# ygjwd12345/UCD

Hardware: AMD Instinct MI355X
Metric: images/sec (whole node) per UCD train step, VOC 15-5 step-1, 513^2 bs=24 (higher is better)
Workload: dtype bf16

## Files before the change

### include/ucd_hip.h

```cpp
#ifndef UCD_HIP_H
#define UCD_HIP_H

#include <stddef.h>
#include <stdint.h>

#ifdef __cplusplus
extern "C" {
#endif

#define UCD_VERSION 100

typedef void* ucd_stream_t;
typedef void* ucd_comm_t;

enum ucd_dtype { UCD_F32 = 0, UCD_BF16 = 1 };
enum ucd_act { UCD_ACT_IDENTITY = 0, UCD_ACT_LEAKY_RELU = 1, UCD_ACT_ELU = 2  };
#define UCD_ACT_MASK 0xff
#define UCD_NORM_ABS_GAMMA 0x100
enum ucd_pixcon_precision { UCD_PIXCON_F32 = 0, UCD_PIXCON_F16 = 1, UCD_PIXCON_F16_SPLIT = 2 };
enum ucd_error {
  UCD_OK = 0,
  UCD_EINVAL = -1,
  UCD_EALIGN = -2,
  UCD_EWORKSPACE = -3,
// ... 247 lines not shown
  const void* residual;  int ldr;
  int out_act;  float out_slope;
  float* partial;
  int accumulate;
  int taps, H, W, dilation;
  const void* side2;  int ld2;
  int stride;
  float* stat_acc;  const float* stat_shift;  float* stat_acc2;
  int stat_rep;
} ucd_conv1x1_desc;

int ucd_conv1x1_row_tiles(int M);
int ucd_conv1x1_stat_replicas(int M);
size_t ucd_conv1x1_stats_partial_bytes(int M, int C);
int ucd_conv1x1(const ucd_conv1x1_desc* desc, ucd_stream_t stream);

int ucd_conv1x1_stats_finalize(const float* partial, int M, int C, const float* weight, float* running_mean,
                               float* running_var, float momentum, float eps, float* buf, float* pack, int flags,
                               ucd_stream_t stream);

int ucd_abn_reduce_partials(const float* partial, int tiles, int C, float* sums, float* sums_copy, const float* weight,
                            int flags, ucd_stream_t stream);

size_t ucd_conv1x1_wgrad_workspace_bytes(int M, int N, int K);
int ucd_conv1x1_wgrad(const void* dy, int ld_dy, const void* a, int lda, int M, int N, int K,
                      const float* in_mean, const float* in_scale, const float* in_shift, int in_act, float in_slope,
                      void* dw, void* workspace, size_t workspace_bytes, ucd_stream_t stream);

int ucd_abn_sync_finalize(const float* gathered, int world, int M, int C, const float* weight, float* running_mean,
                          float* running_var, float momentum, float eps, float* buf, int flags, ucd_stream_t stream);
// ... 84 lines not shown
```

### ucd_amd/csrc/conv1x1.hip

```cpp
#include "common.h"
#include "abn_finalize.h"

namespace ucd {
namespace {

typedef float f32x16 __attribute__((ext_vector_type(16)));
typedef __bf16 bf16x8 __attribute__((ext_vector_type(8)));
typedef __hip_bfloat16 bf16;

constexpr int kThreads = 256;
constexpr int kBM = 128;

constexpr int kBK = 64;
constexpr int kDbStages = 2;
constexpr int kLwStages = 3;

struct Args {
  const bf16* A; int lda;
  const bf16* W; int ldw;
  bf16* Y; int ldy;
  int M, N, K;
  const float *in_mean, *in_scale, *in_shift; int in_act; float in_slope;
  const float *out_mean, *out_scale, *out_shift, *out_invstd;
  const bf16* R; int ldr;
  const bf16* Z; int ldz;
  int out_act; float out_slope;
  float* partial;
  int accumulate;
  int tiles_m, tiles_n;
  int param_off;
  int iH, iW, dil;
  int stride, oW, ohw;
  int a_rows;
  int tiles128;
  float* stat_acc;
  const float* stat_shift;
  float* stat_acc2;
  int stat_rep;
};

__device__ __forceinline__ float act_rt(float z, float slope) { return z > 0.f ? z : z * slope; }
__device__ __forceinline__ float act_grad_rt(float z, float slope) { return z > 0.f ? 1.f : slope; }

__device__ __forceinline__ int swz_fn(int row) { return (row >> 1) & 7; }
__device__ __forceinline__ int swz(int row, int slot) { return row * 128 + ((slot ^ swz_fn(row)) << 4); }

typedef __attribute__((address_space(1))) const void* gptr_t;
typedef __attribute__((address_space(3))) void* lptr_t;


template <int OUT> constexpr int kEpilogueBarriers = 4 + (OUT >= 2 ? 2 : 0);
template <int OUT, int HALVES> constexpr int kEpilogueBarriersH = 2 * HALVES + (OUT >= 2 ? 2 : 0);

__device__ __forceinline__ void live_taps(int m0, int m1, int ohw, int oW, int iH, int dil, int& tap0, int& ntap) {
  tap0 = 0; ntap = 9;
  if (dil <= 1 || m1 - m0 >= ohw) return;
  const int first = m0 % ohw, last = (m1 - 1) % ohw;
  int ymin = first / oW, ymax = last / oW;
  if (first > last) { ymin = 0; ymax = iH - 1; }
  if (ymax < dil) { tap0 = 3; ntap -= 3; }
  if (ymin >= iH - dil) ntap -= 3;
}

template <int BN, bool PRO, int OUT, bool CONV3 = false, bool DB = false>
__global__ __launch_bounds__(kThreads, DB ? 2 : ((PRO || OUT >= 3) && BN == 128 ? 3 : 4)) void conv1x1_kernel(Args p) {
  static_assert(!DB || !PRO, "the double-buffered form has no input transform");
  constexpr int kStage = (kBM + BN) * kBK * 2;
  constexpr int WN = BN / 2;
  constexpr int TN = WN / 32;
  extern __shared__ __attribute__((aligned(1024))) unsigned char smem[];
  unsigned char* As = smem;
  unsigned char* Bs = smem + kBM * kBK * 2;
  float* Ps = reinterpret_cast<float*>(smem + p.param_off);

  const int xcd = blockIdx.x & 7, j = blockIdx.x >> 3;
  const int tm = (j / p.tiles_n) * 8 + xcd, tn = j % p.tiles_n;
  if (tm >= p.tiles_m) return;
  const int m0 = tm * kBM, n0 = tn * BN;
  const int tid = threadIdx.x, lane = tid & 63, wave = __builtin_amdgcn_readfirstlane(tid >> 6);
  const int wm = wave >> 1, wn = wave & 1;

// ... 6 lines not shown
      for (int r = 0; r < 16; ++r) acc[a][b][r] = 0.f;

  constexpr int RPC = 1024 / (kBK * 2), SPR = kBK / 8;
  constexpr int CA = kBM / RPC / 4, CB = BN / RPC / 4;
  const bf16* ga[CA];
  const bf16* gb[CB];
  int py[CA], px[CA], pimg[CA], pslot[CA];
#pragma unroll
  for (int i = 0; i < CA; ++i) {
    const int row = RPC * (wave * CA + i) + lane / SPR;
    const int slot = ((lane % SPR) ^ swz_fn(row)) << 3;
    ga[i] = p.A + (size_t)min(m0 + row, p.M - 1) * p.lda + slot;
    if (CONV3 || p.stride > 1) {
      const int m = m0 + row;
      const int mm = min(m, p.M - 1);
      const int b = mm / p.ohw, rem = mm - b * p.ohw;
      const int oy = rem / p.oW, ox = rem - oy * p.oW;
      py[i] = m < p.M ? oy * p.stride : -(1 << 20);
      px[i] = ox * p.stride;
      pimg[i] = b * p.iH * p.iW;
      pslot[i] = slot;
      if (!CONV3) ga[i] = p.A + (size_t)(pimg[i] + oy * p.stride * p.iW + px[i]) * p.lda + slot;
    }
  }
#pragma unroll
  for (int i = 0; i < CB; ++i) {
    const int row = RPC * (wave * CB + i) + lane / SPR;
    gb[i] = p.W + (size_t)(n0 + row) * p.ldw + (((lane % SPR) ^ swz_fn(row)) << 3);
  }
  const int ks = tid & 7, srow = tid >> 3;
  const bf16* arow[4];
#pragma unroll
  for (int i = 0; i < 4; ++i) arow[i] = p.A + (size_t)min(m0 + srow + 32 * i, p.M - 1) * p.lda + ks * 8;

  if (PRO) {
    for (int k = tid; k < p.K; k += kThreads) {
      Ps[k] = p.in_mean[k];
      Ps[p.K + k] = p.in_scale[k];
      Ps[2 * p.K + k] = p.in_shift ? p.in_shift[k] : 0.f;
    }
    __syncthreads();
  }
  const int fr = lane & 31, fh = lane >> 5;
  const int kpt = p.K / kBK;
  int tap0 = 0, ntap = 9;
  if (CONV3 && p.stride == 1) live_taps(m0, min(m0 + kBM, p.M), p.ohw, p.oW, p.iH, p.dil, tap0, ntap);
  const int nk = CONV3 ? ntap * kpt : kpt;
  uint4 ra[4];
  if (PRO) {
#pragma unroll
    for (int i = 0; i < 4; ++i) ra[i] = *reinterpret_cast<const uint4*>(arow[i]);
  }
  const auto rsW = __builtin_amdgcn_make_buffer_rsrc((void*)p.W, 0, (int)((size_t)p.N * p.ldw * 2), 0x00020000);
  const auto rsA1 = __builtin_amdgcn_make_buffer_rsrc((void*)p.A, 0, (int)((size_t)p.a_rows * p.lda * 2), 0x00020000);
  unsigned boff[CB], a1off[CA];
#pragma unroll
  for (int i = 0; i < CB; ++i) boff[i] = (unsigned)((const char*)gb[i] - (const char*)p.W);
#pragma unroll
  for (int i = 0; i < CA; ++i) a1off[i] = (unsigned)((const char*)ga[i] - (const char*)p.A);
  const auto rsA = __builtin_amdgcn_make_buffer_rsrc((void*)p.A, 0, CONV3 ? (int)((size_t)p.a_rows * p.lda * 2) : 0, 0x00020000);
  constexpr unsigned kOOB = 0x7FFFFFF0u;
  unsigned aoff[CA];
  int atap = -1;
  auto set_tap = [&](int tap) {
    const int dy = (tap / 3 - 1) * p.dil, dx = (tap % 3 - 1) * p.dil;
#pragma unroll
    for (int i = 0; i < CA; ++i) {
      const int yy = py[i] + dy, xx = px[i] + dx;
      const bool ok = (unsigned)yy < (unsigned)p.iH && (unsigned)xx < (unsigned)p.iW;
      aoff[i] = ok ? (unsigned)(((pimg[i] + yy * p.iW + xx) * p.lda + pslot[i]) * 2) : kOOB;
    }
    atap = tap;
  };
  auto fill3 = [&](int kb, unsigned char* Ad, unsigned char* Bd) {
    const int kt = CONV3 ? kb / kpt : 0, tap = tap0 + kt;
    const int k0 = (kb - kt * kpt) * kBK;
    if (CONV3) {
      if (tap != atap) set_tap(tap);
#pragma unroll
      for (int i = 0; i < CA; ++i)
        __builtin_amdgcn_raw_ptr_buffer_load_lds(rsA, (lptr_t)(Ad + (wave * CA + i) * 1024), 16, (int)aoff[i], k0 * 2, 0, 0);
    } else {
#pragma unroll
      for (int i = 0; i < CA; ++i)
        __builtin_amdgcn_raw_ptr_buffer_load_lds(rsA1, (lptr_t)(Ad + (wave * CA + i) * 1024), 16, (int)a1off[i], k0 * 2, 0, 0);
    }
#pragma unroll
    for (int i = 0; i < CB; ++i)
      __builtin_amdgcn_raw_ptr_buffer_load_lds(rsW, (lptr_t)(Bd + (wave * CB + i) * 1024), 16, (int)boff[i], (tap * p.K + k0) * 2, 0, 0);
  };
  if (DB) {
#pragma unroll
    for (int st = 0; st < kDbStages - 1; ++st)
      if (st < nk) fill3(st, As + st * kStage, Bs + st * kStage);
  }
  for (int kb = 0; kb < nk; ++kb) {
    const int kt = CONV3 ? kb / kpt : 0, tap = tap0 + kt;
    const int k0 = (kb - kt * kpt) * kBK;
    const int wk0 = CONV3 ? tap * p.K + k0 : k0;
    if (kb) {
      if (DB) {
        asm volatile("s_waitcnt lgkmcnt(0)" ::: "memory");
        __builtin_amdgcn_s_barrier();
      } else {
        __syncthreads();
      }
    }
    const unsigned char* Ac = As + (DB ? (kb & (kDbStages - 1)) * kStage : 0);
    const unsigned char* Bc = Bs + (DB ? (kb & (kDbStages - 1)) * kStage : 0);
    if (DB) {
      if (kb + kDbStages - 1 < nk) {
        const int st = (kb + kDbStages - 1) & (kDbStages - 1);
// ... 76 lines not shown
#pragma unroll
        for (int a = 0; a < 2; ++a) af[a] = *reinterpret_cast<const bf16x8*>(Ac + swz(wm * 64 + a * 32 + fr, 2 * kk + fh));
#pragma unroll
        for (int b = 0; b < TN; ++b) bfr[b] = *reinterpret_cast<const bf16x8*>(Bc + swz(wn * WN + b * 32 + fr, 2 * kk + fh));
#pragma unroll
        for (int a = 0; a < 2; ++a)
#pragma unroll
          for (int b = 0; b < TN; ++b) acc[a][b] = __builtin_amdgcn_mfma_f32_32x32x16_bf16(af[a], bfr[b], acc[a][b], 0, 0, 0);
      }
    }
  }

#include "conv1x1_epilogue.inc"
}

template <int BM, int BN, int OUT, bool CONV3>
__global__ __launch_bounds__(BM == 64 ? 384 : BM * 4, (BM + BN) * kBK * 2 * kLwStages > 80 * 1024 ? 1 : 2) void conv_lw_kernel(Args p) {
  static_assert(BM == 64 || BM == 128 || BM == 256, "64-, 128- or 256-row workgroup tiles");
  static_assert(BM != 64 || BN == 64, "the 64-row form runs its epilogue on 128 threads: 64-column tiles");
  constexpr int NC = BM / 32, NL = BM == 64 ? 4 : BM / 32;
  constexpr int kStage = (BM + BN) * kBK * 2;
  constexpr int WN = BN / 2, TN = WN / 32;
  extern __shared__ __attribute__((aligned(1024))) unsigned char smem[];
  unsigned char* As = smem;
  unsigned char* Bs = smem + BM * kBK * 2;
  const int xcd = blockIdx.x & 7, j = blockIdx.x >> 3;
  const int tmw = (j / p.tiles_n) * 8 + xcd, tn = j % p.tiles_n;
  if (tmw >= p.tiles_m) return;
  const int m0w = tmw * BM, n0 = tn * BN;
  const int tid = threadIdx.x, lane = tid & 63, wave = __builtin_amdgcn_readfirstlane(tid >> 6);
  const int kpt = p.K / kBK;
  int tap0 = 0, ntap = 9;
  if (CONV3 && p.stride == 1) live_taps(m0w, min(m0w + BM, p.M), p.ohw, p.oW, p.iH, p.dil, tap0, ntap);
  const int nk = CONV3 ? ntap * kpt : kpt;

  if (wave >= NC) {
    const int lw = wave - NC;
    const int m0 = m0w;
    constexpr int RPC = 1024 / (kBK * 2), SPR = kBK / 8;
    constexpr int CA = BM / RPC / NL, CB = BN / RPC / NL;
    int py[CA], px[CA], pimg[CA], pslot[CA];
    unsigned a1off[CA], boff[CB];
#pragma unroll
    for (int i = 0; i < CA; ++i) {
      const int row = RPC * (lw * CA + i) + lane / SPR;
      const int slot = ((lane % SPR) ^ swz_fn(row)) << 3;
      a1off[i] = (unsigned)(((size_t)min(m0 + row, p.M - 1) * p.lda + slot) * 2);
      if (CONV3 || p.stride > 1) {
        const int m = m0 + row;
        const int mm = min(m, p.M - 1);
        const int b = mm / p.ohw, rem = mm - b * p.ohw;
        const int oy = rem / p.oW, ox = rem - oy * p.oW;
        py[i] = m < p.M ? oy * p.stride : -(1 << 20);
        px[i] = ox * p.stride;
        pimg[i] = b * p.iH * p.iW;
        pslot[i] = slot;
        if (!CONV3) a1off[i] = (unsigned)(((size_t)(pimg[i] + oy * p.stride * p.iW + px[i]) * p.lda + slot) * 2);
      }
    }
#pragma unroll
    for (int i = 0; i < CB; ++i) {
      const int row = RPC * (lw * CB + i) + lane / SPR;
      boff[i] = (unsigned)(((size_t)(n0 + row) * p.ldw + (((lane % SPR) ^ swz_fn(row)) << 3)) * 2);
    }
    const auto rsW = __builtin_amdgcn_make_buffer_rsrc((void*)p.W, 0, (int)((size_t)p.N * p.ldw * 2), 0x00020000);
    const auto rsA = __builtin_amdgcn_make_buffer_rsrc((void*)p.A, 0, (int)((size_t)p.a_rows * p.lda * 2), 0x00020000);
    constexpr unsigned kOOB = 0x7FFFFFF0u;
    unsigned aoff[CA];
    int atap = -1;
    auto set_tap = [&](int tap) {
      const int dy = (tap / 3 - 1) * p.dil, dx = (tap % 3 - 1) * p.dil;
#pragma unroll
      for (int i = 0; i < CA; ++i) {
        const int yy = py[i] + dy, xx = px[i] + dx;
        const bool ok = (unsigned)yy < (unsigned)p.iH && (unsigned)xx < (unsigned)p.iW;
        aoff[i] = ok ? (unsigned)(((pimg[i] + yy * p.iW + xx) * p.lda + pslot[i]) * 2) : kOOB;
      }
      atap = tap;
    };
    auto fill = [&](int kb, int st) {
      unsigned char* Ad = As + st * kStage;
      unsigned char* Bd = Bs + st * kStage;
      const int kt = CONV3 ? kb / kpt : 0, tap = tap0 + kt;
      const int k0 = (kb - kt * kpt) * kBK;
      if (CONV3) {
        if (tap != atap) set_tap(tap);
#pragma unroll
        for (int i = 0; i < CA; ++i)
          __builtin_amdgcn_raw_ptr_buffer_load_lds(rsA, (lptr_t)(Ad + (lw * CA + i) * 1024), 16, (int)aoff[i], k0 * 2, 0, 0);
      } else {
#pragma unroll
        for (int i = 0; i < CA; ++i)
          __builtin_amdgcn_raw_ptr_buffer_load_lds(rsA, (lptr_t)(Ad + (lw * CA + i) * 1024), 16, (int)a1off[i], k0 * 2, 0, 0);
      }
#pragma unroll
      for (int i = 0; i < CB; ++i)
        __builtin_amdgcn_raw_ptr_buffer_load_lds(rsW, (lptr_t)(Bd + (lw * CB + i) * 1024), 16, (int)boff[i], (tap * p.K + k0) * 2, 0, 0);
    };
// ... 348 lines not shown
        if (co + j < Co) q[j] = tmp[j];
    }
  }
}

int pick_wgrad_chunks(int M, int N, int K) {
  const int tiles = (N / 128) * (K / 128);
  int chunks = (512 + tiles - 1) / tiles;
  const int max_chunks = (M + 255) / 256;
  if (chunks > max_chunks) chunks = max_chunks;
  if (chunks < 1) chunks = 1;
  return chunks;
}


template <int BN, int OUT, bool CONV3>
int launch_db(int pipe, int grid, hipStream_t s, const Args& a, const char* fn) {
  constexpr size_t kOut = (size_t)64 * (BN + 4) * 4, kRed = (size_t)(kThreads / (BN / 8)) * 2 * BN * 4;
  auto lds_of = [&](int nst) {
    size_t l = (size_t)(kBM + BN) * kBK * 2 * nst;
    if (l < kOut) l = kOut;
    if (l < kRed) l = kRed;
    return l;
  };
  if (pipe == 5) {
    if constexpr (OUT <= 2 && BN == 128) {
      Args b = a;
      b.tiles_m = ceil_div(a.M, 256);
      const int grid256 = ceil_div(b.tiles_m, 8) * 8 * b.tiles_n;
      size_t lds = (size_t)(256 + BN) * kBK * 2 * kLwStages;
      if (lds < kOut) lds = kOut;
      UCD_TRY_LDS((conv_lw_kernel<256, BN, OUT, CONV3>), (int)lds);
      conv_lw_kernel<256, BN, OUT, CONV3><<<grid256, 1024, lds, s>>>(b);
      return 0;
    }
    pipe = 0;
  }
  if (pipe == 7) {
    if constexpr (BN == 64) {
      Args b = a;
      b.tiles_m = ceil_div(a.M, 64);
      const int grid64 = ceil_div(b.tiles_m, 8) * 8 * b.tiles_n;
      const size_t lds64 = (size_t)(64 + BN) * kBK * 2 * kLwStages;
      conv_lw_kernel<64, BN, OUT, CONV3><<<grid64, 384, lds64, s>>>(b);
      return 0;
    }
    pipe = 4;
  }
  if (pipe == 4) {
    const size_t lds = lds_of(kLwStages);
    UCD_TRY_LDS((conv_lw_kernel<128, BN, OUT, CONV3>), (int)lds);
    conv_lw_kernel<128, BN, OUT, CONV3><<<grid, 2 * kThreads, lds, s>>>(a);
    return 0;
  }
  conv1x1_kernel<BN, false, OUT, CONV3, true><<<grid, kThreads, lds_of(kDbStages), s>>>(a);
  return 0;
}

template <int BN, bool CONV3>
int launch_db_out(int out_mode, int pipe, int grid, hipStream_t s, const Args& a, const char* fn) {
  switch (out_mode) {
    case 0: return launch_db<BN, 0, CONV3>(pipe, grid, s, a, fn);
    case 1: return launch_db<BN, 1, CONV3>(pipe, grid, s, a, fn);
    case 2: return launch_db<BN, 2, CONV3>(pipe, grid, s, a, fn);
    case 3: return launch_db<BN, 3, CONV3>(pipe, grid, s, a, fn);
    default:
      if constexpr (CONV3) {
        set_error("%s: out_mode 4 belongs to the 1x1 products", fn);
        return UCD_EINVAL;
      } else {
        return launch_db<BN, 4, false>(pipe, grid, s, a, fn);
      }
  }
}

int forced_pipe() {
  static const int forced = [] {
    const char* e = getenv("UCD_CONV_PIPE");
    return !e || !*e || !strcmp(e, "auto") ? -1 : !strcmp(e, "2x64") ? 0 : !strcmp(e, "lw64") ? 4 : !strcmp(e, "lw256") ? 5 : -2;
  }();
  return forced;
}

int pick_pipe(int M, int tiles_n, int BN, int nk64, int out_mode) {
  if (forced_pipe() >= 0) return forced_pipe();
  const long long wg128 = (long long)ceil_div(M, 128) * tiles_n, wg256 = (long long)ceil_div(M, 256) * tiles_n;
  if (wg128 <= 256 && nk64 >= 4) return 4;
  if (BN == 128 && out_mode <= 2 && wg256 <= 256 && nk64 >= 4) return 5;
  return 0;
}

}
}

using namespace ucd;

extern "C" {

int ucd_conv1x1_row_tiles(int M) { return ceil_div(M, kBM); }

int ucd_conv1x1_stat_replicas(int M) {
  const int tiles = ceil_div(M, kBM);
  int r = 1;
  while (r < 64 && tiles > 64 * r) r *= 2;
// ... 42 lines not shown
  Args a;
  a.A = (const bf16*)d->a; a.lda = d->lda; a.W = (const bf16*)d->w; a.ldw = d->ldw; a.Y = (bf16*)d->y; a.ldy = d->ldy;
  a.M = d->M; a.N = d->N; a.K = d->K;
  a.in_mean = d->in_mean; a.in_scale = d->in_scale; a.in_shift = d->in_shift;
  a.in_act = d->in_act & UCD_ACT_MASK; a.in_slope = a.in_act == UCD_ACT_IDENTITY ? 1.f : d->in_slope;
  a.out_mean = d->out_mean; a.out_scale = d->out_scale; a.out_shift = d->out_shift; a.out_invstd = d->out_invstd;
  a.R = (const bf16*)d->residual; a.ldr = d->ldr;
  a.Z = (const bf16*)d->side2; a.ldz = d->ld2;
  a.out_act = d->out_act & UCD_ACT_MASK; a.out_slope = a.out_act == UCD_ACT_IDENTITY ? 1.f : d->out_slope;
  a.partial = d->partial; a.accumulate = d->accumulate;
  a.iH = d->H; a.iW = d->W; a.dil = d->dilation;
  a.tiles128 = ceil_div(d->M, 128);
  a.stride = stride; a.oW = oW > 0 ? oW : 1; a.ohw = oH * oW > 0 ? oH * oW : 1; a.a_rows = (int)a_rows;
  a.stat_acc = d->out_mode >= 2 ? d->stat_acc : nullptr; a.stat_shift = d->stat_shift; a.stat_acc2 = d->stat_acc2;
  a.stat_rep = d->stat_rep > 1 ? d->stat_rep : 1;
  UCD_REQUIRE((a.stat_rep & (a.stat_rep - 1)) == 0, UCD_EINVAL, "%s: stat_rep must be a power of two", fn);
  UCD_REQUIRE(!a.stat_acc || d->out_mode != 2 || (d->stat_shift && aligned16(d->stat_shift)), UCD_EINVAL,
              "%s: out_mode 2 with stat_acc needs a 16-byte aligned stat_shift", fn);
  static const int bn64_below = getenv("UCD_CONV_BN64_TILES") ? atoi(getenv("UCD_CONV_BN64_TILES")) : 128;
  const int BN = (d->N % 128 == 0 && (long long)ceil_div(d->M, kBM) * (d->N / 128) > bn64_below) ? 128 : 64;
  a.tiles_m = ceil_div(d->M, kBM); a.tiles_n = d->N / BN;
  const int grid = ceil_div(a.tiles_m, 8) * 8 * a.tiles_n;
  hipStream_t s = (hipStream_t)stream;
  const bool db = ((conv3 || !d->in_scale) && (long long)ceil_div(d->M, kBM) * (d->N / BN) <= 640) || (d->out_mode == 4 && BN == 128);
  const size_t lds_main = (size_t)(kBM + BN) * 128 * (db ? 2 : 1), lds_out = (size_t)64 * (BN + 4) * 4;
  size_t lds = lds_main > lds_out ? lds_main : lds_out;
  const size_t lds_red = (size_t)(kThreads / (BN / 8)) * 2 * BN * 4;
  if (lds_red > lds) lds = lds_red;
  const bool pro = d->in_scale != nullptr;
  a.param_off = (int)align_up(lds, 16);
  if (pro) lds = a.param_off + (size_t)3 * d->K * sizeof(float);
  UCD_REQUIRE(lds <= 64 * 1024, UCD_EUNSUPPORTED, "%s: K = %d is too wide for the fused input transform", fn, d->K);
  int pipe = db ? pick_pipe(d->M, a.tiles_n, BN, (conv3 ? 9 : 1) * (d->K / 64), d->out_mode) : 0;
  static const int lw64_below = getenv("UCD_CONV_LW64_TILES") ? atoi(getenv("UCD_CONV_LW64_TILES")) : 128;
  if (db && !pro && pipe == 4 && BN == 64 && (long long)a.tiles_m * a.tiles_n <= lw64_below && (d->out_mode < 2 || a.stat_acc)) pipe = 7;
  if (db && !pro) {
    int rc;
    if (conv3) rc = BN == 128 ? launch_db_out<128, true>(d->out_mode, pipe, grid, s, a, fn) : launch_db_out<64, true>(d->out_mode, pipe, grid, s, a, fn);
    else rc = BN == 128 ? launch_db_out<128, false>(d->out_mode, pipe, grid, s, a, fn) : launch_db_out<64, false>(d->out_mode, pipe, grid, s, a, fn);
    if (rc) return rc;
    return check_launch(fn);
  }
#define UCD_C1_OUT(BNV, PROV)                                                   \
  switch (d->out_mode) {                                                        \
    case 0: conv1x1_kernel<BNV, PROV, 0><<<grid, kThreads, lds, s>>>(a); break; \
    case 1: conv1x1_kernel<BNV, PROV, 1><<<grid, kThreads, lds, s>>>(a); break; \
    case 2: conv1x1_kernel<BNV, PROV, 2><<<grid, kThreads, lds, s>>>(a); break; \
    case 3: conv1x1_kernel<BNV, PROV, 3><<<grid, kThreads, lds, s>>>(a); break; \
    default: conv1x1_kernel<BNV, false, 4><<<grid, kThreads, lds, s>>>(a); break; \
  }
#define UCD_C3_OUT(BNV)                                                                        \
  switch (d->out_mode) {                                                                       \
    case 0: conv1x1_kernel<BNV, false, 0, true, false><<<grid, kThreads, lds, s>>>(a); break;  \
    case 1: conv1x1_kernel<BNV, false, 1, true, false><<<grid, kThreads, lds, s>>>(a); break;  \
    case 2: conv1x1_kernel<BNV, false, 2, true, false><<<grid, kThreads, lds, s>>>(a); break;  \
    case 4: UCD_REQUIRE(false, UCD_EINVAL, "%s: out_mode 4 belongs to the 1x1 products", fn);  \
    default: conv1x1_kernel<BNV, false, 3, true, false><<<grid, kThreads, lds, s>>>(a); break; \
  }
  if (conv3) {
    if (BN == 128) { UCD_C3_OUT(128) } else { UCD_C3_OUT(64) }
  } else if (BN == 128) {
    if (pro) { UCD_C1_OUT(128, true) } else { UCD_C1_OUT(128, false) }
  } else {
    if (pro) { UCD_C1_OUT(64, true) } else { UCD_C1_OUT(64, false) }
  }
#undef UCD_C3_OUT
#undef UCD_C1_OUT
  return check_launch(fn);
}

size_t ucd_conv1x1_stats_partial_bytes(int M, int C) { return (size_t)ceil_div(M, kBM) * 3 * C * sizeof(float); }

int ucd_conv1x1_stats_finalize(const float* partial, int M, int C, const float* weight, float* running_mean,
                               float* running_var, float momentum, float eps, float* buf, float* pack, int flags,
                               ucd_stream_t stream) {
  static const char* fn = "ucd_conv1x1_stats_finalize";
  UCD_REQUIRE(partial && buf && M > 0 && C > 0, UCD_EINVAL, "%s: bad arguments", fn);
  const int tiles = ceil_div(M, kBM);
  float *sums = buf, *kshift = buf + 2 * C, *mean = buf + 3 * C, *invstd = buf + 4 * C, *scale = buf + 5 * C;
  FinalizeArgs fin{kshift, weight, running_mean, running_var, mean, invstd, scale, (float)M, momentum, eps, pack,
                   (flags & UCD_NORM_ABS_GAMMA) != 0};
  hipStream_t s = (hipStream_t)stream;
  if (pack)
// ... 71 lines not shown
```

### ucd_amd/csrc/conv1x1_epilogue.inc

```
#ifndef UCD_EPI_ACTIVE
#define UCD_EPI_ACTIVE true
#define UCD_EPI_ACTIVE_DEFAULTED
#endif
#ifndef UCD_EPI_TILE_OK
#define UCD_EPI_TILE_OK true
#define UCD_EPI_TILE_OK_DEFAULTED
#endif
#ifndef UCD_EPI_THREADS
#define UCD_EPI_THREADS kThreads
#define UCD_EPI_HALVES 2
#define UCD_EPI_THREADS_DEFAULTED
#endif
  constexpr int CP = BN + 4;
  float* Cs = reinterpret_cast<float*>(smem);
  constexpr int CPR = BN / 8;
  constexpr int RPT = 64 * CPR / (UCD_EPI_THREADS);
  constexpr int RSTEP = (UCD_EPI_THREADS) / CPR;
  const int c8 = tid % CPR, r0 = tid / CPR;
  const int ncol = n0 + c8 * 8;
  Pack8 em, es, eb, ei;
  if (OUT == 3) {
    em = load_f8(p.out_mean + ncol);
    es = load_f8(p.out_scale + ncol);
    eb = load_f8(p.out_shift + ncol);
// ... 13 lines not shown
    em = load_f8(p.out_mean + ncol);
    ei = load_f8(p.out_invstd + ncol);
  }
  Pack8 kshift, s1, s2;
#pragma unroll
  for (int j = 0; j < 4; ++j) { kshift.p[j] = f32x2{0.f, 0.f}; s1.p[j] = f32x2{0.f, 0.f}; s2.p[j] = f32x2{0.f, 0.f}; }
  const bool has_side = ((OUT == 0 || OUT == 4) && p.accumulate) || (OUT == 1 && p.R != nullptr) || OUT == 3;
  const bf16* sp = (OUT == 0 || OUT == 4) ? p.Y : p.R;
  const int lds_ = (OUT == 0 || OUT == 4) ? p.ldy : p.ldr;
#pragma unroll
  for (int half = 0; half < (UCD_EPI_HALVES); ++half) {
    uint4 side[RPT], side_y[OUT == 4 ? RPT : 1], side_z[OUT == 4 ? RPT : 1];
    if (has_side && UCD_EPI_ACTIVE) {
#pragma unroll
      for (int i = 0; i < RPT; ++i)
        side[i] = *reinterpret_cast<const uint4*>(sp + (size_t)min(m0 + half * 64 + r0 + RSTEP * i, p.M - 1) * lds_ + ncol);
    }
    if (OUT == 4) {
#pragma unroll
      for (int i = 0; i < RPT; ++i) {
        const size_t row = (size_t)min(m0 + half * 64 + r0 + RSTEP * i, p.M - 1);
        side_y[i] = *reinterpret_cast<const uint4*>(p.R + row * p.ldr + ncol);
        side_z[i] = *reinterpret_cast<const uint4*>(p.Z + row * p.ldz + ncol);
      }
    }
    __syncthreads();
    if (wm == half) {
#pragma unroll
      for (int a = 0; a < 2; ++a)
#pragma unroll
        for (int b = 0; b < TN; ++b)
// ... 75 lines not shown
#pragma unroll
          for (int j = 0; j < 4; ++j) v.p[j] += sv.p[j];
        }
#pragma unroll
        for (int j = 0; j < 4; ++j) o.p[j] = leaky_grad2(v.p[j], yv.p[j], p.out_slope);
        packed = pack8(o);
        if (live) {
          const Pack8 q = unpack8(packed);
#pragma unroll
          for (int j = 0; j < 4; ++j) {
            s1.p[j] += q.p[j];
            s2.p[j] += q.p[j] * ((zv.p[j] - em.p[j]) * ei.p[j]);
          }
        }
      }
      if (live) *reinterpret_cast<uint4*>(p.Y + (size_t)grow * p.ldy + ncol) = packed;
    }
  }
  if (OUT >= 2) {
    __syncthreads();
    float* red = Cs;
    if (UCD_EPI_ACTIVE) {
#pragma unroll
      for (int j = 0; j < 4; ++j) {
        *reinterpret_cast<f32x2*>(red + (r0 * 2 + 0) * BN + c8 * 8 + 2 * j) = s1.p[j];
        *reinterpret_cast<f32x2*>(red + (r0 * 2 + 1) * BN + c8 * 8 + 2 * j) = s2.p[j];
      }
    }
    __syncthreads();
    if (tid < 2 * BN && UCD_EPI_TILE_OK) {
      const int which = tid / BN, col = tid % BN;
// ... 38 lines not shown
```

### ucd_amd/hip.py

```python
from __future__ import annotations

import ctypes as C
import os

import torch

_HERE = os.path.dirname(os.path.abspath(__file__))
LIB_PATH = os.path.join(_HERE, "libucd_hip.so")

F32, BF16 = 0, 1
ACT_IDENTITY, ACT_LEAKY_RELU, ACT_ELU = 0, 1, 2
ACT_CODES = {"identity": ACT_IDENTITY, "leaky_relu": ACT_LEAKY_RELU, "elu": ACT_ELU}
ACT_MASK = 0xFF
NORM_ABS_GAMMA = 0x100
PIX_TILE = 128
PIXCON_LD = 256
PIXCON_F32, PIXCON_F16, PIXCON_F16_SPLIT = 0, 1, 2
KD_UNBIASED, KD_PLAIN = 0, 1
SEG_FORMS = {1: "pk<16,8>", 2: "pk<20,4>", 3: "pk<12,12>", 4: "reg<24,16>", 5: "reg<24,24>", 6: "wide/fixed", 7: "wide/f32"}
PIXCON_PATHS = {1: "f32", 2: "f32/wide", 3: "f16/planned", 4: "f16/split"}
PIXCON_PRECISION = {"f32": PIXCON_F32, "fp32": PIXCON_F32, "f16": PIXCON_F16, "fp16": PIXCON_F16,
                    "f16_split": PIXCON_F16_SPLIT}


# ... 68 lines not shown
                               _f, _i, _i, _f, _p]),
    "ucd_abn_forward": (_i, [_p, _i, _p, _i, _p, _i, _i, _i, _i, _p, _i, _p, _p, _p, _p, _f, _f, _i, _p, _p, _i, _f, _p, _z, _p]),
    "ucd_abn_backward": (_i, [_p, _i, _p, _i, _p, _i, _p, _i, _p, _i, _i, _i, _i, _p, _i, _p, _p, _p, _p, _p, _p, _f, _i, _i,
                              _i, _f, _p, _z, _p]),
    "ucd_plane_sum": (_i, [_p, _i, _i, _i, _i, _i, _f, _p, _p]),
    "ucd_window_mean_workspace_bytes": (_z, [_i, _i, _i, _i, _i]),
    "ucd_window_mean": (_i, [_p, _i, _i, _i, _i, _i, _i, _i, _i, _p, _i, _p, _z, _p]),
    "ucd_attmap_workspace_bytes": (_z, [_i, _i]),
    "ucd_attmap": (_i, [_p, _i, _p, _i, _i, _i, _i, _i, _p, _z, _p]),
    "ucd_attn_mse_workspace_bytes": (_z, [_i, _i]),
    "ucd_attn_mse": (_i, [_p, _i, _p, _i, _i, _i, _i, _i, _f, _p, _p, _i, _p, _z, _p]),
    "ucd_conv1x1_row_tiles": (_i, [_i]),
    "ucd_conv1x1_stats_partial_bytes": (_z, [_i, _i]),
    "ucd_conv1x1": (_i, [C.POINTER(Conv1x1Desc), _p]),
    "ucd_conv1x1_stats_finalize": (_i, [_p, _i, _i, _p, _p, _p, _f, _f, _p, _p, _i, _p]),
    "ucd_abn_reduce_partials": (_i, [_p, _i, _i, _p, _p, _p, _i, _p]),
    "ucd_conv1x1_wgrad_workspace_bytes": (_z, [_i, _i, _i]),
    "ucd_conv1x1_wgrad": (_i, [_p, _i, _p, _i, _i, _i, _i, _p, _p, _p, _i, _f, _p, _p, _z, _p]),
    "ucd_abn_sync_finalize": (_i, [_p, _i, _i, _i, _p, _p, _p, _f, _f, _p, _i, _p]),
    "ucd_stem_pooled_size": (_i, [_i]),
    "ucd_stem_pool_workspace_bytes": (_z, [_i]),
    "ucd_stem_apply_pool": (_i, [_p, _i, _i, _i, _i, _p, _p, _p, _i, _f, _p, _p, _p]),
    "ucd_stem_pool_backward": (_i, [_p, _p, _p, _i, _i, _i, _i, _p, _p, _p, _p, _p, _p, _f, _i, _f, _p, _p, _z, _i, _p]),
    "ucd_conv_wgrad_workspace_bytes": (_z, [_i, _i, _i, _i]),
    "ucd_conv_wgrad": (_i, [_p, _i, _p, _i, _i, _i, _i, _i, _i, _i, _i, _p, _p, _i, _p, _z, _p]),
    "ucd_stem_conv7x7": (_i, [_p, C.c_longlong, C.c_longlong, C.c_longlong, C.c_longlong, _i, _i, _i, _p, _p, _p]),
    "ucd_stem_conv_pool": (_i, [_p, C.c_longlong, C.c_longlong, C.c_longlong, C.c_longlong, _i, _i, _i, _p, _p, _p, _p, _i, _f, _p, _p]),
    "ucd_conv_wgrad_strided": (_i, [_p, _i, _p, _i, _i, _i, _i, _i, _i, _i, _i, _i, _p, _p, _i, _p, _z, _p]),
    "ucd_conv_wgrad_ex": (_i, [_p, _i, _p, _i, _i, _i, _i, _i, _i, _i, _i, _i, _p, _p, _i, _p, _z, _i, _p]),
    "ucd_conv_wgrad_defer": (_i, [_i]),
# ... 250 lines not shown
        _check(rc, "ucd_abn_backward")


def pixcon_loss_plan(BHW, K, precision="f32", use_prob=True, temperature=0.07):
    lib = load()
    prec = PIXCON_PRECISION[precision] if isinstance(precision, str) else int(precision)
    path, chunk, n1, n2 = C.c_int(0), C.c_int(0), C.c_int(0), C.c_int(0)
    l1, l2, wsb = C.c_size_t(0), C.c_size_t(0), C.c_size_t(0)
    _check(lib.ucd_pixcon_loss_plan(int(BHW), int(K), prec, int(bool(use_prob)), float(temperature), C.addressof(path),
                                    C.addressof(chunk), C.addressof(n1), C.addressof(n2), C.addressof(l1), C.addressof(l2),
                                    C.addressof(wsb)), "ucd_pixcon_loss_plan")
    return {"path": PIXCON_PATHS[path.value], "class_chunk": chunk.value, "nsplit1": n1.value, "nsplit2": n2.value,
            "lds_sweep1": l1.value, "lds_sweep2": l2.value, "workspace_bytes": wsb.value}


_gemm_ready = None


def _loaded_library_path(fragment):
    try:
        with open("/proc/self/maps") as f:
            for line in f:
                if fragment in line:
                    return line.split()[-1]
    except OSError:
        pass
    return ""


def gemm_available():
# ... 373 lines not shown
```

### ucd_amd/switches.py

```python
from __future__ import annotations

import os

DEFAULTS = {
    "UCD_FUSED_CONV1X1": "1",
    "UCD_BWD_LINK": "1",
    "UCD_BLOCK_LINK": "1",
    "UCD_PROJ_ALIAS": "1",
    "UCD_DGRAD_VIA_FWD": "1",
    "UCD_LIB_GEMM_WIDE": "0",
    "UCD_OWN3X3_MIN_TILES": "1",
    "UCD_OWN3X3_WIDE": "1",
    "UCD_OWN_STRIDED": "1",
    "UCD_OWN_WGRAD": "1",
    "UCD_F32_OWN_CONV": "0",
    "UCD_OWN_HEADS": "1",
    "UCD_OWN_STEM": "1",
    "UCD_WGRAD3": "1",
    "UCD_CONV_PIPE": "auto",
    "UCD_CONV_BN64_TILES": "128",
    "UCD_CONV_LW64_TILES": "128",
    "UCD_WGRAD_DEFER": "1",
    "UCD_WGRAD_STREAM": "1",
    "UCD_CONV3_MIN_ROWS": "0",
    "UCD_STAT_ATOMIC": "1",
    "UCD_SEG_PK": "1",
    "UCD_SEG_KD_EX": "1",
    "UCD_FUSED_LDE": "1",
    "UCD_STEM_EVAL_FUSED": "1",
    "UCD_STEM_FOLD": "1",
    "UCD_ABN_NODE": "1",
    "UCD_SGD": "hip",
    "UCD_STEP_GRAPH": "auto",
    "UCD_TEACHER_OVERLAP": "1",
    "UCD_DIRECT_RCCL": "1",
    "UCD_IPC_SYNC": "auto",
    "UCD_IPC_TIMEOUT_MS": "60000",
    "UCD_DDP_LATE_COPY": "1",
# ... 33 lines not shown
```

Before: 867.7.

## Reorder dilated 3x3 conv rows by border class to skip dead taps

For dilated stride-1 3x3 convolutions with the plain output mode, output pixels are permuted so that pixels sharing the same set of in-bounds taps sit together. Each tile then gets a per-tile tap bitmask, and the kernel iterates only the live taps instead of the coarse row-range pruning. The plan is built on the host, cached on the device, and the epilogue scatters rows back through the permutation. This adds gather/scatter indirection, less contiguous output writes, and a one-time host plan cost in exchange for fewer MFMA k-steps at image borders with large dilation.

```diff
diff --git a/include/ucd_hip.h b/include/ucd_hip.h
--- a/include/ucd_hip.h
+++ b/include/ucd_hip.h
@@ -285,6 +285,11 @@
 int ucd_conv1x1_stat_replicas(int M);
 size_t ucd_conv1x1_stats_partial_bytes(int M, int C);
 int ucd_conv1x1(const ucd_conv1x1_desc* desc, ucd_stream_t stream);
+
+int ucd_conv3_tap_plan(int B, int H, int W, int dilation, int tile_rows, int* perm, int* masks, int* n_classes);
+int ucd_conv3_tap_classes(int mode);
+int ucd_conv3_tap_plans_resident(void);
+int ucd_conv3_tap_stats(long long* launches, int* last_tile_rows, int* last_class_ordered);
 
 int ucd_conv1x1_stats_finalize(const float* partial, int M, int C, const float* weight, float* running_mean,
                                float* running_var, float momentum, float eps, float* buf, float* pack, int flags,
diff --git a/ucd_amd/csrc/conv1x1.hip b/ucd_amd/csrc/conv1x1.hip
--- a/ucd_amd/csrc/conv1x1.hip
+++ b/ucd_amd/csrc/conv1x1.hip
@@ -1,5 +1,9 @@
 #include "common.h"
 #include "abn_finalize.h"
+#include "conv3_taps.h"
+#include <algorithm>
+#include <mutex>
+#include <vector>
 
 namespace ucd {
 namespace {
@@ -37,7 +41,11 @@
   const float* stat_shift;
   float* stat_acc2;
   int stat_rep;
+  const int* perm;
+  const int* masks;
 };
+
+#define UCD_EPI_ROW(r) (RT ? p.perm[min((r), p.M - 1)] : (r))
 
 __device__ __forceinline__ float act_rt(float z, float slope) { return z > 0.f ? z : z * slope; }
 __device__ __forceinline__ float act_grad_rt(float z, float slope) { return z > 0.f ? 1.f : slope; }
@@ -62,9 +70,10 @@
   if (ymin >= iH - dil) ntap -= 3;
 }
 
-template <int BN, bool PRO, int OUT, bool CONV3 = false, bool DB = false>
+template <int BN, bool PRO, int OUT, bool CONV3 = false, bool DB = false, bool RT = false>
 __global__ __launch_bounds__(kThreads, DB ? 2 : ((PRO || OUT >= 3) && BN == 128 ? 3 : 4)) void conv1x1_kernel(Args p) {
   static_assert(!DB || !PRO, "the double-buffered form has no input transform");
+  static_assert(!RT || (CONV3 && OUT == 0 && !PRO), "class-ordered rows: the plain 3x3 product");
   constexpr int kStage = (kBM + BN) * kBK * 2;
   constexpr int WN = BN / 2;
   constexpr int TN = WN / 32;
@@ -101,7 +110,8 @@
     if (CONV3 || p.stride > 1) {
       const int m = m0 + row;
       const int mm = min(m, p.M - 1);
-      const int b = mm / p.ohw, rem = mm - b * p.ohw;
+      const int pix = RT ? p.perm[mm] : mm;
+      const int b = pix / p.ohw, rem = pix - b * p.ohw;
       const int oy = rem / p.oW, ox = rem - oy * p.oW;
       py[i] = m < p.M ? oy * p.stride : -(1 << 20);
       px[i] = ox * p.stride;
@@ -131,8 +141,19 @@
   const int fr = lane & 31, fh = lane >> 5;
   const int kpt = p.K / kBK;
   int tap0 = 0, ntap = 9;
-  if (CONV3 && p.stride == 1) live_taps(m0, min(m0 + kBM, p.M), p.ohw, p.oW, p.iH, p.dil, tap0, ntap);
+  unsigned trem = 0;
+  if constexpr (RT) { trem = (unsigned)p.masks[tm]; ntap = __builtin_popcount(trem); }
+  else if (CONV3 && p.stride == 1) live_taps(m0, min(m0 + kBM, p.M), p.ohw, p.oW, p.iH, p.dil, tap0, ntap);
   const int nk = CONV3 ? ntap * kpt : kpt;
+  int akt = -1, ctap = 0;
+  auto tap_of = [&](int kt) {
+    if constexpr (RT) {
+      if (kt != akt) { ctap = __builtin_ctz(trem); trem &= trem - 1; akt = kt; }
+      return ctap;
+    } else {
+      return tap0 + kt;
+    }
+  };
   uint4 ra[4];
   if (PRO) {
 #pragma unroll
@@ -160,7 +181,7 @@
     atap = tap;
   };
   auto fill3 = [&](int kb, unsigned char* Ad, unsigned char* Bd) {
-    const int kt = CONV3 ? kb / kpt : 0, tap = tap0 + kt;
+    const int kt = CONV3 ? kb / kpt : 0, tap = tap_of(kt);
     const int k0 = (kb - kt * kpt) * kBK;
     if (CONV3) {
       if (tap != atap) set_tap(tap);
@@ -182,7 +203,7 @@
       if (st < nk) fill3(st, As + st * kStage, Bs + st * kStage);
   }
   for (int kb = 0; kb < nk; ++kb) {
-    const int kt = CONV3 ? kb / kpt : 0, tap = tap0 + kt;
+    const int kt = CONV3 ? kb / kpt : 0, tap = DB ? 0 : tap_of(kt);
     const int k0 = (kb - kt * kpt) * kBK;
     const int wk0 = CONV3 ? tap * p.K + k0 : k0;
     if (kb) {
@@ -289,10 +310,11 @@
 #include "conv1x1_epilogue.inc"
 }
 
-template <int BM, int BN, int OUT, bool CONV3>
+template <int BM, int BN, int OUT, bool CONV3, bool RT = false>
 __global__ __launch_bounds__(BM == 64 ? 384 : BM * 4, (BM + BN) * kBK * 2 * kLwStages > 80 * 1024 ? 1 : 2) void conv_lw_kernel(Args p) {
   static_assert(BM == 64 || BM == 128 || BM == 256, "64-, 128- or 256-row workgroup tiles");
   static_assert(BM != 64 || BN == 64, "the 64-row form runs its epilogue on 128 threads: 64-column tiles");
+  static_assert(!RT || (CONV3 && OUT == 0), "class-ordered rows: the plain 3x3 product");
   constexpr int NC = BM / 32, NL = BM == 64 ? 4 : BM / 32;
   constexpr int kStage = (BM + BN) * kBK * 2;
   constexpr int WN = BN / 2, TN = WN / 32;
@@ -306,7 +328,9 @@
   const int tid = threadIdx.x, lane = tid & 63, wave = __builtin_amdgcn_readfirstlane(tid >> 6);
   const int kpt = p.K / kBK;
   int tap0 = 0, ntap = 9;
-  if (CONV3 && p.stride == 1) live_taps(m0w, min(m0w + BM, p.M), p.ohw, p.oW, p.iH, p.dil, tap0, ntap);
+  unsigned trem = 0;
+  if constexpr (RT) { trem = (unsigned)p.masks[tmw]; ntap = __builtin_popcount(trem); }
+  else if (CONV3 && p.stride == 1) live_taps(m0w, min(m0w + BM, p.M), p.ohw, p.oW, p.iH, p.dil, tap0, ntap);
   const int nk = CONV3 ? ntap * kpt : kpt;
 
   if (wave >= NC) {
@@ -324,7 +348,8 @@
       if (CONV3 || p.stride > 1) {
         const int m = m0 + row;
         const int mm = min(m, p.M - 1);
-        const int b = mm / p.ohw, rem = mm - b * p.ohw;
+        const int pix = RT ? p.perm[mm] : mm;
+        const int b = pix / p.ohw, rem = pix - b * p.ohw;
         const int oy = rem / p.oW, ox = rem - oy * p.oW;
         py[i] = m < p.M ? oy * p.stride : -(1 << 20);
         px[i] = ox * p.stride;
@@ -353,10 +378,15 @@
       }
       atap = tap;
     };
+    int akt = -1, ctap = 0;
+    auto next_tap = [&](int kt) {
+      if (kt != akt) { ctap = __builtin_ctz(trem); trem &= trem - 1; akt = kt; }
+      return ctap;
+    };
     auto fill = [&](int kb, int st) {
       unsigned char* Ad = As + st * kStage;
       unsigned char* Bd = Bs + st * kStage;
-      const int kt = CONV3 ? kb / kpt : 0, tap = tap0 + kt;
+      const int kt = CONV3 ? kb / kpt : 0, tap = RT ? next_tap(kt) : tap0 + kt;
       const int k0 = (kb - kt * kpt) * kBK;
       if (CONV3) {
         if (tap != atap) set_tap(tap);
@@ -735,7 +765,7 @@
 }
 
 
-template <int BN, int OUT, bool CONV3>
+template <int BN, int OUT, bool CONV3, bool RT = false>
 int launch_db(int pipe, int grid, hipStream_t s, const Args& a, const char* fn) {
   constexpr size_t kOut = (size_t)64 * (BN + 4) * 4, kRed = (size_t)(kThreads / (BN / 8)) * 2 * BN * 4;
   auto lds_of = [&](int nst) {
@@ -751,8 +781,8 @@
       const int grid256 = ceil_div(b.tiles_m, 8) * 8 * b.tiles_n;
       size_t lds = (size_t)(256 + BN) * kBK * 2 * kLwStages;
       if (lds < kOut) lds = kOut;
-      UCD_TRY_LDS((conv_lw_kernel<256, BN, OUT, CONV3>), (int)lds);
-      conv_lw_kernel<256, BN, OUT, CONV3><<<grid256, 1024, lds, s>>>(b);
+      UCD_TRY_LDS((conv_lw_kernel<256, BN, OUT, CONV3, RT>), (int)lds);
+      conv_lw_kernel<256, BN, OUT, CONV3, RT><<<grid256, 1024, lds, s>>>(b);
       return 0;
     }
     pipe = 0;
@@ -763,25 +793,29 @@
       b.tiles_m = ceil_div(a.M, 64);
       const int grid64 = ceil_div(b.tiles_m, 8) * 8 * b.tiles_n;
       const size_t lds64 = (size_t)(64 + BN) * kBK * 2 * kLwStages;
-      conv_lw_kernel<64, BN, OUT, CONV3><<<grid64, 384, lds64, s>>>(b);
+      conv_lw_kernel<64, BN, OUT, CONV3, RT><<<grid64, 384, lds64, s>>>(b);
       return 0;
     }
     pipe = 4;
   }
   if (pipe == 4) {
     const size_t lds = lds_of(kLwStages);
-    UCD_TRY_LDS((conv_lw_kernel<128, BN, OUT, CONV3>), (int)lds);
-    conv_lw_kernel<128, BN, OUT, CONV3><<<grid, 2 * kThreads, lds, s>>>(a);
+    UCD_TRY_LDS((conv_lw_kernel<128, BN, OUT, CONV3, RT>), (int)lds);
+    conv_lw_kernel<128, BN, OUT, CONV3, RT><<<grid, 2 * kThreads, lds, s>>>(a);
     return 0;
   }
-  conv1x1_kernel<BN, false, OUT, CONV3, true><<<grid, kThreads, lds_of(kDbStages), s>>>(a);
+  conv1x1_kernel<BN, false, OUT, CONV3, true, RT><<<grid, kThreads, lds_of(kDbStages), s>>>(a);
   return 0;
 }
 
 template <int BN, bool CONV3>
 int launch_db_out(int out_mode, int pipe, int grid, hipStream_t s, const Args& a, const char* fn) {
   switch (out_mode) {
-    case 0: return launch_db<BN, 0, CONV3>(pipe, grid, s, a, fn);
+    case 0:
+      if constexpr (CONV3) {
+        if (a.perm) return launch_db<BN, 0, true, true>(pipe, grid, s, a, fn);
+      }
+      return launch_db<BN, 0, CONV3>(pipe, grid, s, a, fn);
     case 1: return launch_db<BN, 1, CONV3>(pipe, grid, s, a, fn);
     case 2: return launch_db<BN, 2, CONV3>(pipe, grid, s, a, fn);
     case 3: return launch_db<BN, 3, CONV3>(pipe, grid, s, a, fn);
@@ -809,6 +843,74 @@
   if (wg128 <= 256 && nk64 >= 4) return 4;
   if (BN == 128 && out_mode <= 2 && wg256 <= 256 && nk64 >= 4) return 5;
   return 0;
+}
+
+int tile_rows_of(bool db_launch, int pipe, int BN, int out_mode) {
+  if (!db_launch) return kBM;
+  if (pipe == 5 && BN == 128 && out_mode <= 2) return 256;
+  if (pipe == 7 && BN == 64) return 64;
+  return kBM;
+}
+
+int g_tap_classes = -1;
+std::mutex g_tap_mutex;
+int tap_classes_mode() {
+  std::lock_guard<std::mutex> lock(g_tap_mutex);
+  if (g_tap_classes < 0) {
+    const char* e = getenv("UCD_CONV3_TAP_CLASSES");
+    g_tap_classes = e && !strcmp(e, "0") ? 0 : e && !strcmp(e, "2") ? 2 : 1;
+  }
+  return g_tap_classes;
+}
+
+struct TapPlan { int dev, B, H, W, d, rows; int* perm; int* masks; int max_on, max_off; };
+std::vector<TapPlan> g_tap_plans;
+constexpr size_t kMaxTapPlans = 64;
+long long g_tap_launches = 0;
+int g_tap_last_rows = 0, g_tap_last_rt = 0;
+
+int heaviest_raster_tile(int B, int H, int W, int d, int rows) {
+  const int hw = H * W, M = B * hw;
+  int best = 0;
+  for (int m0 = 0; m0 < M; m0 += rows) {
+    const int m1 = m0 + rows < M ? m0 + rows : M;
+    int nt = 9;
+    if (m1 - m0 < hw) {
+      const int first = m0 % hw, last = (m1 - 1) % hw;
+      int ymin = first / W, ymax = last / W;
+      if (first > last) { ymin = 0; ymax = H - 1; }
+      if (ymax < d) nt -= 3;
+      if (ymin >= H - d) nt -= 3;
+    }
+    if (nt > best) best = nt;
+  }
+  return best;
+}
+
+const TapPlan* tap_plan_get(int B, int H, int W, int d, int rows, hipStream_t s) {
+  int dev = 0;
+  if (hipGetDevice(&dev) != hipSuccess) { (void)hipGetLastError(); return nullptr; }
+  std::lock_guard<std::mutex> lock(g_tap_mutex);
+  for (const TapPlan& t : g_tap_plans)
+    if (t.dev == dev && t.B == B && t.H == H && t.W == W && t.d == d && t.rows == rows) return &t;
+  if (g_tap_plans.size() >= kMaxTapPlans) return nullptr;
+  hipStreamCaptureStatus cap = hipStreamCaptureStatusNone;
+  if (hipStreamIsCapturing(s, &cap) != hipSuccess || cap != hipStreamCaptureStatusNone) { (void)hipGetLastError(); return nullptr; }
+  const int M = B * H * W, tiles = ceil_div(M, rows);
+  std::vector<int32_t> host((size_t)M + tiles);
+  conv3_tap_plan_fill(B, H, W, d, rows, host.data(), host.data() + M);
+  int* devp = nullptr;
+  if (hipMalloc((void**)&devp, host.size() * sizeof(int32_t)) != hipSuccess) { (void)hipGetLastError(); return nullptr; }
+  if (hipMemcpy(devp, host.data(), host.size() * sizeof(int32_t), hipMemcpyHostToDevice) != hipSuccess) {
+    (void)hipGetLastError();
+    (void)hipFree(devp);
+    return nullptr;
+  }
+  int max_on = 0;
+  for (int t = 0; t < tiles; ++t) max_on = std::max(max_on, __builtin_popcount((unsigned)host[(size_t)M + t]));
+  g_tap_plans.reserve(kMaxTapPlans);
+  g_tap_plans.push_back(TapPlan{dev, B, H, W, d, rows, devp, devp + M, max_on, heaviest_raster_tile(B, H, W, d, rows)});
+  return &g_tap_plans.back();
 }
 
 }
@@ -881,6 +983,7 @@
   a.stride = stride; a.oW = oW > 0 ? oW : 1; a.ohw = oH * oW > 0 ? oH * oW : 1; a.a_rows = (int)a_rows;
   a.stat_acc = d->out_mode >= 2 ? d->stat_acc : nullptr; a.stat_shift = d->stat_shift; a.stat_acc2 = d->stat_acc2;
   a.stat_rep = d->stat_rep > 1 ? d->stat_rep : 1;
+  a.perm = nullptr; a.masks = nullptr;
   UCD_REQUIRE((a.stat_rep & (a.stat_rep - 1)) == 0, UCD_EINVAL, "%s: stat_rep must be a power of two", fn);
   UCD_REQUIRE(!a.stat_acc || d->out_mode != 2 || (d->stat_shift && aligned16(d->stat_shift)), UCD_EINVAL,
               "%s: out_mode 2 with stat_acc needs a 16-byte aligned stat_shift", fn);
@@ -901,6 +1004,20 @@
   int pipe = db ? pick_pipe(d->M, a.tiles_n, BN, (conv3 ? 9 : 1) * (d->K / 64), d->out_mode) : 0;
   static const int lw64_below = getenv("UCD_CONV_LW64_TILES") ? atoi(getenv("UCD_CONV_LW64_TILES")) : 128;
   if (db && !pro && pipe == 4 && BN == 64 && (long long)a.tiles_m * a.tiles_n <= lw64_below && (d->out_mode < 2 || a.stat_acc)) pipe = 7;
+  if (conv3 && stride == 1 && d->dilation > 1 && d->out_mode == 0) {
+    const int mode = tap_classes_mode(), rows = tile_rows_of(db && !pro, pipe, BN, d->out_mode);
+    const TapPlan* tp = mode ? tap_plan_get(d->M / (d->H * d->W), d->H, d->W, d->dilation, rows, s) : nullptr;
+    if (tp && mode == 1 && rows == 64 && tp->max_on >= tp->max_off) {
+      int dev = 0, cus = 0;
+      if (hipGetDevice(&dev) == hipSuccess && hipDeviceGetAttribute(&cus, hipDeviceAttributeMultiprocessorCount, dev) == hipSuccess &&
+          (long long)ceil_div(d->M, rows) * a.tiles_n <= cus)
+        tp = nullptr;
+    }
+    if (tp) { a.perm = tp->perm; a.masks = tp->masks; }
+    std::lock_guard<std::mutex> lock(g_tap_mutex);
+    g_tap_launches += tp != nullptr;
+    g_tap_last_rows = rows; g_tap_last_rt = tp != nullptr;
+  }
   if (db && !pro) {
     int rc;
     if (conv3) rc = BN == 128 ? launch_db_out<128, true>(d->out_mode, pipe, grid, s, a, fn) : launch_db_out<64, true>(d->out_mode, pipe, grid, s, a, fn);
@@ -918,7 +1035,10 @@
   }
 #define UCD_C3_OUT(BNV)                                                                        \
   switch (d->out_mode) {                                                                       \
-    case 0: conv1x1_kernel<BNV, false, 0, true, false><<<grid, kThreads, lds, s>>>(a); break;  \
+    case 0:                                                                                    \
+      if (a.perm) conv1x1_kernel<BNV, false, 0, true, false, true><<<grid, kThreads, lds, s>>>(a); \
+      else conv1x1_kernel<BNV, false, 0, true, false><<<grid, kThreads, lds, s>>>(a);           \
+      break;                                                                                   \
     case 1: conv1x1_kernel<BNV, false, 1, true, false><<<grid, kThreads, lds, s>>>(a); break;  \
     case 2: conv1x1_kernel<BNV, false, 2, true, false><<<grid, kThreads, lds, s>>>(a); break;  \
     case 4: UCD_REQUIRE(false, UCD_EINVAL, "%s: out_mode 4 belongs to the 1x1 products", fn);  \
@@ -934,6 +1054,37 @@
 #undef UCD_C3_OUT
 #undef UCD_C1_OUT
   return check_launch(fn);
+}
+
+int ucd_conv3_tap_classes(int mode) {
+  const int cur = tap_classes_mode();
+  if (mode < 0) return cur;
+  std::lock_guard<std::mutex> lock(g_tap_mutex);
+  g_tap_classes = mode >= 2 ? 2 : mode;
+  return g_tap_classes;
+}
+
+int ucd_conv3_tap_stats(long long* launches, int* last_tile_rows, int* last_class_ordered) {
+  std::lock_guard<std::mutex> lock(g_tap_mutex);
+  if (launches) *launches = g_tap_launches;
+  if (last_tile_rows) *last_tile_rows = g_tap_last_rows;
+  if (last_class_ordered) *last_class_ordered = g_tap_last_rt;
+  return 0;
+}
+
+int ucd_conv3_tap_plan(int B, int H, int W, int dilation, int tile_rows, int* perm, int* masks, int* n_classes) {
+  static const char* fn = "ucd_conv3_tap_plan";
+  UCD_REQUIRE(B > 0 && H > 0 && W > 0 && dilation >= 1 && perm && masks, UCD_EINVAL, "%s: bad arguments", fn);
+  UCD_REQUIRE(tile_rows == 64 || tile_rows == 128 || tile_rows == 256, UCD_EINVAL, "%s: tile_rows must be 64, 128 or 256", fn);
+  UCD_REQUIRE((long long)B * H * W < 0x7FFFFFFF, UCD_EUNSUPPORTED, "%s: more than 2^31 rows", fn);
+  const int n = conv3_tap_plan_fill(B, H, W, dilation, tile_rows, perm, masks);
+  if (n_classes) *n_classes = n;
+  return 0;
+}
+
+int ucd_conv3_tap_plans_resident(void) {
+  std::lock_guard<std::mutex> lock(g_tap_mutex);
+  return (int)g_tap_plans.size();
 }
 
 size_t ucd_conv1x1_stats_partial_bytes(int M, int C) { return (size_t)ceil_div(M, kBM) * 3 * C * sizeof(float); }
diff --git a/ucd_amd/csrc/conv1x1_epilogue.inc b/ucd_amd/csrc/conv1x1_epilogue.inc
--- a/ucd_amd/csrc/conv1x1_epilogue.inc
+++ b/ucd_amd/csrc/conv1x1_epilogue.inc
@@ -5,6 +5,9 @@
 #ifndef UCD_EPI_TILE_OK
 #define UCD_EPI_TILE_OK true
 #define UCD_EPI_TILE_OK_DEFAULTED
+#endif
+#ifndef UCD_EPI_ROW
+#define UCD_EPI_ROW(r) (r)
 #endif
 #ifndef UCD_EPI_THREADS
 #define UCD_EPI_THREADS kThreads
@@ -51,7 +54,7 @@
     if (has_side && UCD_EPI_ACTIVE) {
 #pragma unroll
       for (int i = 0; i < RPT; ++i)
-        side[i] = *reinterpret_cast<const uint4*>(sp + (size_t)min(m0 + half * 64 + r0 + RSTEP * i, p.M - 1) * lds_ + ncol);
+        side[i] = *reinterpret_cast<const uint4*>(sp + (size_t)UCD_EPI_ROW(min(m0 + half * 64 + r0 + RSTEP * i, p.M - 1)) * lds_ + ncol);
     }
     if (OUT == 4) {
 #pragma unroll
@@ -157,7 +160,7 @@
           }
         }
       }
-      if (live) *reinterpret_cast<uint4*>(p.Y + (size_t)grow * p.ldy + ncol) = packed;
+      if (live) *reinterpret_cast<uint4*>(p.Y + (size_t)UCD_EPI_ROW(grow) * p.ldy + ncol) = packed;
     }
   }
   if (OUT >= 2) {
diff --git a/ucd_amd/csrc/conv3_taps.h b/ucd_amd/csrc/conv3_taps.h
--- /dev/null
+++ b/ucd_amd/csrc/conv3_taps.h
@@ -0,0 +1,45 @@
+#pragma once
+#include <cstdint>
+
+namespace ucd {
+
+inline int conv3_axis_class(int v, int n, int d) { return (v - d >= 0 ? 1 : 0) | (v + d < n ? 2 : 0); }
+
+inline unsigned conv3_axis_taps(int cls) { return 2u | (cls & 1 ? 1u : 0u) | (cls & 2 ? 4u : 0u); }
+
+inline unsigned conv3_class_mask(int cy, int cx) {
+  const unsigned ty = conv3_axis_taps(cy), tx = conv3_axis_taps(cx);
+  unsigned m = 0;
+  for (int kh = 0; kh < 3; ++kh)
+    for (int kw = 0; kw < 3; ++kw)
+      if ((ty >> kh & 1) && (tx >> kw & 1)) m |= 1u << (kh * 3 + kw);
+  return m;
+}
+
+inline int conv3_tap_plan_fill(int B, int H, int W, int d, int tile_rows, int32_t* perm, int32_t* masks) {
+  const int HW = H * W, M = B * HW;
+  int count[16] = {0}, order[16], start[16];
+  for (int y = 0; y < H; ++y)
+    for (int x = 0; x < W; ++x) count[conv3_axis_class(y, H, d) * 4 + conv3_axis_class(x, W, d)] += B;
+  int n = 0;
+  for (int c = 0; c < 16; ++c)
+    if (count[c]) order[n++] = c;
+  auto taps = [](int c) { return __builtin_popcount(conv3_class_mask(c >> 2, c & 3)); };
+  for (int i = 1; i < n; ++i)
+    for (int j = i; j > 0 && taps(order[j]) > taps(order[j - 1]); --j) { const int t = order[j]; order[j] = order[j - 1]; order[j - 1] = t; }
+  int at = 0;
+  for (int i = 0; i < n; ++i) { start[order[i]] = at; at += count[order[i]]; }
+  const int tiles = (M + tile_rows - 1) / tile_rows;
+  for (int t = 0; t < tiles; ++t) masks[t] = 0;
+  for (int b = 0; b < B; ++b)
+    for (int y = 0; y < H; ++y)
+      for (int x = 0; x < W; ++x) {
+        const int cy = conv3_axis_class(y, H, d), cx = conv3_axis_class(x, W, d);
+        const int r = start[cy * 4 + cx]++;
+        perm[r] = b * HW + y * W + x;
+        masks[r / tile_rows] |= (int32_t)conv3_class_mask(cy, cx);
+      }
+  return n;
+}
+
+}
diff --git a/ucd_amd/hip.py b/ucd_amd/hip.py
--- a/ucd_amd/hip.py
+++ b/ucd_amd/hip.py
@@ -106,6 +106,10 @@
     "ucd_conv1x1_stats_partial_bytes": (_z, [_i, _i]),
     "ucd_conv1x1": (_i, [C.POINTER(Conv1x1Desc), _p]),
     "ucd_conv1x1_stats_finalize": (_i, [_p, _i, _i, _p, _p, _p, _f, _f, _p, _p, _i, _p]),
+    "ucd_conv3_tap_plan": (_i, [_i, _i, _i, _i, _i, _p, _p, _p]),
+    "ucd_conv3_tap_classes": (_i, [_i]),
+    "ucd_conv3_tap_plans_resident": (_i, []),
+    "ucd_conv3_tap_stats": (_i, [_p, _p, _p]),
     "ucd_abn_reduce_partials": (_i, [_p, _i, _i, _p, _p, _p, _i, _p]),
     "ucd_conv1x1_wgrad_workspace_bytes": (_z, [_i, _i, _i]),
     "ucd_conv1x1_wgrad": (_i, [_p, _i, _p, _i, _i, _i, _i, _p, _p, _p, _i, _f, _p, _p, _z, _p]),
@@ -386,6 +390,31 @@
             "lds_sweep1": l1.value, "lds_sweep2": l2.value, "workspace_bytes": wsb.value}
 
 
+def conv3_tap_plan(B, H, W, dilation, tile_rows):
+    import numpy as np
+    M = int(B) * int(H) * int(W)
+    perm = np.empty(M, dtype=np.int32)
+    masks = np.empty((M + int(tile_rows) - 1) // int(tile_rows), dtype=np.int32)
+    n = C.c_int(0)
+    _check(load().ucd_conv3_tap_plan(int(B), int(H), int(W), int(dilation), int(tile_rows), perm.ctypes.data, masks.ctypes.data,
+                                     C.addressof(n)), "ucd_conv3_tap_plan")
+    return perm, masks, n.value
+
+
+def conv3_tap_classes(mode=None):
+    return load().ucd_conv3_tap_classes(-1 if mode is None else int(mode))
+
+
+def conv3_tap_stats():
+    n, rows, rt = C.c_longlong(0), C.c_int(0), C.c_int(0)
+    load().ucd_conv3_tap_stats(C.addressof(n), C.addressof(rows), C.addressof(rt))
+    return n.value, rows.value, bool(rt.value)
+
+
+def conv3_tap_plans_resident():
+    return load().ucd_conv3_tap_plans_resident()
+
+
 _gemm_ready = None
 
 
diff --git a/ucd_amd/switches.py b/ucd_amd/switches.py
--- a/ucd_amd/switches.py
+++ b/ucd_amd/switches.py
@@ -22,6 +22,7 @@
     "UCD_CONV_LW64_TILES": "128",
     "UCD_WGRAD_DEFER": "1",
     "UCD_WGRAD_STREAM": "1",
+    "UCD_CONV3_TAP_CLASSES": "1",
     "UCD_CONV3_MIN_ROWS": "0",
     "UCD_STAT_ATOMIC": "1",
     "UCD_SEG_PK": "1",
```

After: 877.0 (median of 6 runs). 1.01x the previous value.
